# JeffWang987/MVSTER

Measured on AMD Instinct MI355X. Metric: depth-maps/sec (DTU 512×640, 5-view, 4-stage) at 1/2/4/8 MI355X, higher is better.
Workload: dtype f32; 1 GPU; DTU mid 512x640, 5 views, 4-stage cascade 8/8/4/4 hyp, B=1 eval, 1 depth map(s) per step per GPU; launch=hipGraph replay, parallelism=replicas x1, depth_maps_in_flight_per_gpu=2

## Files before the change

### include/mvster_hip.h

```cpp
#ifndef MVSTER_HIP_H
#define MVSTER_HIP_H

#ifdef __cplusplus
extern "C" {
#endif

#define MVSTER_OK 0
#define MVSTER_ERR_NULL (-1)
#define MVSTER_ERR_SHAPE (-2)
#define MVSTER_ERR_UNSUPPORTED (-3)
#define MVSTER_ERR_LAUNCH (-4)

int mvster_relative_projection(const float* proj_matrices, float* rt, int B, int N, void* stream);

int mvster_relative_projection_multi(const float* const* proj_matrices, int nstage, float* rt, int B, int N,
                                     void* stream);

int mvster_pack_images(const float* const* imgs, int N, float* out, int B, int H, int W, void* stream);

int mvster_pack_images_u8(const unsigned char* imgs, float* out, int V, int H, int W, void* stream);

int mvster_load_pack_images_u8(const unsigned char* buf, long buf_bytes, const int* desc_host, const int* desc, const void* tables,
                               long table_words, float* out, unsigned char* out_u8, int V, int Hd, int Wd, void* stream);

int mvster_forward_prologue(const float* const* imgs, int N, float* packed, int B, int H, int W,
                            const float* const* proj_matrices, int nstage, float* rt, const float* depth_values, int ndv,
                            float* hypo, int D, int h, int w, int inverse, void* stream);

int mvster_warp_agg_fwd(const float* ref_feat, const float* src_feat, const float* rt, const float* hypo,
                        float* out, float* wsum_out, int B, int NV, int C, int G, int D, int h, int w, int Hs,
                        int Ws, long ref_batch_stride, long src_view_stride, long src_batch_stride, int group_cor,
                        int attn_fuse_d, float attn_temp, int variant, void* stream);

int mvster_warp_agg_fwd_indexed(const float* store, const int* views, const float* rt, const float* hypo, float* out,
                                float* wsum_out, int V, int B, int NV, int C, int G, int D, int h, int w, int group_cor,
                                int attn_fuse_d, float attn_temp, int variant, void* stream);

int mvster_warp_agg_fwd_counted(const float* ref_feat, const float* src_feat, const float* rt, const float* hypo,
                                float* out, float* wsum_out, int B, int NV, int C, int G, int D, int h, int w, int Hs,
                                int Ws, long ref_batch_stride, long src_view_stride, long src_batch_stride, int group_cor,
                                int attn_fuse_d, float attn_temp, int variant, const int* nsrc, void* stream);
int mvster_warp_agg_fwd_indexed_counted(const float* store, const int* views, const float* rt, const float* hypo, float* out,
                                        float* wsum_out, int V, int B, int NV, int C, int G, int D, int h, int w,
                                        int group_cor, int attn_fuse_d, float attn_temp, int variant, const int* nsrc,
                                        void* stream);

int mvster_gather_views(const float* store, const int* views, float* out, int V, int B, int N, long map_floats, void* stream);

int mvster_warp_agg_fwd_sched(const float* ref_feat, const float* src_feat, const float* rt, const float* inv_min,
                              const float* inv_max, const float* depth_values, int ndv, float* hypo_out, float* out,
                              float* wsum_out, int B, int NV, int C, int G, int D, int h, int w, int Hs, int Ws,
                              long ref_batch_stride, long src_view_stride, long src_batch_stride, int attn_fuse_d,
                              float attn_temp, int mode, void* stream);

int mvster_warp_agg_bwd(const float* ref_feat, const float* src_feat, const float* rt, const float* hypo,
                        const float* out, const float* wsum, const float* grad_out, float* grad_ref,
                        float* grad_src, float* windows, int* win_org, int B, int NV, int C, int G, int D, int h, int w,
                        int Hs, int Ws, long ref_batch_stride, long src_view_stride, long src_batch_stride, int group_cor,
                        int attn_fuse_d, float attn_temp, void* stream);
int mvster_warp_agg_bwd_scratch(int B, int NV, int C, int G, int D, int h, int w, int attn_fuse_d, long* window_floats,
                                long* origin_ints);

int mvster_warp_agg_bwd_sorted_scratch(int B, int NV, int C, int D, int h, int w, int Hs, int Ws, long* rec_floats, long* ints);
int mvster_warp_agg_bwd_sorted(const float* ref_feat, const float* src_feat, const float* rt, const float* hypo,
                               const float* out, const float* wsum, const float* grad_out, float* grad_ref, float* grad_src,
                               float* rec, int* ints, int B, int NV, int C, int G, int D, int h, int w, int Hs, int Ws,
                               long ref_batch_stride, long src_view_stride, long src_batch_stride, int group_cor,
                               int attn_fuse_d, float attn_temp, void* stream);

int mvster_init_range(const float* depth_values, int ndv, float* out, int B, int D, int h, int w, int inverse,
                      void* stream);

int mvster_schedule_inverse_range(const float* inv_min, const float* inv_max, float* out, int B, int D, int h,
                                  int w, void* stream);

int mvster_schedule_range(const float* cur_depth, const float* interval, float* out, int B, int D, int h, int w,
                          void* stream);

int mvster_select_depth(const float* logits, const float* feat, const float* prob_w, const float* prob_b, int CF,
                        const float* hypo, float* attn, float* depth, float* conf, float* inv_min, float* inv_max,
                        float* logits_out, int B, int D, int h, int w, float split_itv, void* stream);

int mvster_select_depth_bwd(const float* attn, const float* gattn, const float* feat, const float* prob_w, float* dfeat,
                            float* partial, int B, int D, int h, int w, int CF, void* stream);

int mvster_upsample_bilinear(const float* in, float* out, int B, int hi, int wi, int ho, int wo, void* stream);

int mvster_upsample_bilinear_multi(const float* const* ins, float* const* outs, const int* his, const int* wis, int n, int B,
                                   int ho, int wo, void* stream);

int mvster_conv_mfma(const float* in, const float* wpk, const float* scale, const float* shift, const float* skip,
                     const float* zeros, const float* prob_w, const float* prob_b, float* out, const int* geom,
                     int ngeom, const long* woff, int cin, int mt, int nt, int variant, void* stream);

int mvster_conv_small(const float* in, const float* w, const float* scale, const float* shift, const float* skip,
                      float* out, int NB, int H, int W, int cin, int relu, void* stream);

int mvster_conv_narrow(const float* in, const float* w, const float* scale, const float* shift, const float* skip,
                       float* out, int NB, int H, int W, int cin, int relu, int mt, int wpc, void* stream);

int mvster_conv_narrow4(const float* in, const float* w, const float* scale, const float* shift, float* out, int NB, int H,
                        int W, int relu, int mt, int wpc, void* stream);

int mvster_conv_narrow_pair(const float* in, const float* w1, const float* scale1, const float* shift1, const float* w2,
                            const float* scale2, const float* shift2, float* out, int NB, int H, int W, int relu1, int relu2,
                            int wpc, void* stream);

int mvster_deconv_small(const float* in, const float* w, const float* scale, const float* shift, const float* skip,
                        const float* prob_w, const float* prob_b, float* out, int NB, int Hi, int Wi, int cin,
                        int cout, int relu, void* stream);

int mvster_deconv_select(const float* in, const float* w, const float* scale, const float* shift, const float* skip,
                         const float* prob_w, const float* prob_b, const float* hypo, float* attn, float* depth, float* conf,
                         float* inv_min, float* inv_max, float* logits_out, int B, int D, int Hi, int Wi, int cin, int relu,
                         float split_itv, void* stream);

int mvster_fpn_tail_gather(const float* G, const float* vb, float* P, float* workspace, int NB, int H, int W,
                           int CO, void* stream);

int mvster_fpn_tail_gather_bwd(const float* gP, float* gG, int NB, int H, int W, int CO, int pitch, void* stream);

int mvster_fpn_lateral_up(const float* x, const float* A, const float* bias, const float* q, float* out, int NB,
                          int H, int W, int CI, int CO, void* stream);

int mvster_fpn_tail_fused(const float* x, const float* A, const float* bias, const float* q, const float* vb, float* P,
                          int NB, int H, int W, int CI, void* stream);

int mvster_pack_conv_weights(const float* w, float* wpk, int cout, int cin, int cin_pad, int kd, int kh, int kw, long s_n,
                             long s_c, long s_z, long s_y, long s_x, int flip, void* stream);

int mvster_pack_wino_weights(const float* w, float* wpk, int cout, int cin, int cin_pad, int kd, long s_n, long s_c, long s_z,
                             long s_y, long s_x, int flip, void* stream);

int mvster_pack_wino_batch(const void* descs, int ndesc, int total_blocks, void* stream);

int mvster_pack_conv_weights_classes(const float* w, float* wpk, int cout, int cin, int cin_pad, int ktot, int nclass,
                                     const int* ntaps, const long* woff, const int* taps, void* stream);

int mvster_conv_wgrad(const float* x, const float* gy, float* partial, int nblk, int B, int Di, int Hi, int Wi, int CI,
                      int Do, int Ho, int Wo, int CO, int kd, int kh, int kw, int sd, int sh, int sw, int pd, int ph,
                      int pw, int packed, void* stream);

int mvster_conv_wgrad_slots(int CI, int CO, int kd, int kh, int kw, int sd, int sh, int sw, int pd, int ph, int pw, int packed);

int mvster_conv_wgrad_finish(const float* partial, float* dw, int nblk, int ngrp, int cop, int width, int ntaps, int cip,
                             int co_lim, int ci_lim, int swap, int flip, void* stream);

int mvster_conv_wgrad_finish_batch(const void* recs, int count, void* stream);

int mvster_bn_relu_fwd(const float* x, const float* scale, const float* shift, const float* skip, float* y, long rows,
                       int C, int relu, int groups, void* stream);
int mvster_bn_slots(long rows, int C, int groups);
int mvster_bn_relu_bwd_reduce(const float* x, const float* gy, const float* scale, const float* shift, const float* mean,
                              const float* rstd, float* partial, float* sums, float* dgamma, float* dbeta, int* ticket,
                              long rows, int C, int relu, int groups, void* stream);
int mvster_bn_relu_bwd_apply(const float* x, const float* gy, const float* scale, const float* shift, const float* mean,
                             const float* rstd, const float* sums, float* dx, long rows, int C, int relu, int groups,
                             int frozen, void* stream);

int mvster_col_sum(const float* x, float* partial, float* out, int* ticket, long rows, int C, void* stream);

int mvster_bn_train_slots(long rows, int C, int groups);
int mvster_bn_train_fwd(const float* x, const float* weight, const float* bias, float* running_mean, float* running_var,
                        long* num_batches_tracked, const float* skip, float* partial, float* y, float* out, long rows, int C,
                        int relu, int groups, float eps, float momentum, void* stream);
int mvster_bn_train_bwd(const float* x, const float* gy, const float* pack, float* partial, float* dgamma, float* dbeta, float* dx,
                        long rows, int C, int relu, int groups, void* stream);

int mvster_upsample2x_cl_fwd(const float* in, float* out, int B, int h, int w, int C, void* stream);
int mvster_upsample2x_cl_bwd(const float* gout, float* gin, int B, int h, int w, int C, void* stream);
int mvster_upsample2x_nearest_cl(const float* in, float* out, int B, int h, int w, int C, int backward, void* stream);

int mvster_sinkhorn(const float* attn, const float* hypo, const float* gt, float* loss_pix, float* jac, int B, int D,
                    long HW, int iters, float eps, void* stream);
int mvster_sinkhorn_continuous(const float* attn, const float* hypo, const float* gt, const float* mask, float* loss_pix,
                               float* jac, int B, int D, long HW, int iters, float eps, void* stream);

int mvster_stage_loss_terms(const float* hypo, const float* gt, const float* mask, const float* loss_pix,
                            const float* mono, float* terms, int B, int D, long HW, int inverse_depth, void* stream);

int mvster_geo_filter(const float* depth_ref, const float* depth_src, const double* ref_mats, const double* view_mats,
                      int* mask_sum, float* depth_sum, unsigned char* view_mask, float* view_depth, float* x_src,
                      float* y_src, int NS, int H, int W, float pix_thres, float rel_thres, void* stream);


int mvster_geo_scene_blocks(int R, int H, int W);

int mvster_geo_scene_filter(const float* depth, const float* confidence, const int* pairs, const int* ref_view,
                            const double* ref_mats, const double* view_mats, int* mask_sum, double* depth_avg,
// ... 78 lines not shown
```

### mvster_amd/_lib.py

```python
import ctypes
import os

_HERE = os.path.dirname(os.path.abspath(__file__))
LIB_PATH = os.environ.get("MVSTER_LIB") or os.path.join(_HERE, "csrc", "libmvster_hip.so")

ERR_NULL, ERR_SHAPE, ERR_UNSUPPORTED, ERR_LAUNCH = -1, -2, -3, -4
ERRORS = {-1: "NULL pointer", -2: "bad shape", -3: "unsupported channel/tile combination", -4: "kernel launch failed"}

_f = ctypes.c_void_p
_i = ctypes.c_int
_l = ctypes.c_long
_fl = ctypes.c_float

SIGNATURES = {
    "mvster_relative_projection": [_f, _f, _i, _i, _f],
    "mvster_relative_projection_multi": [_f, _i, _f, _i, _i, _f],
    "mvster_pack_images": [_f, _i, _f, _i, _i, _i, _f],
    "mvster_pack_images_u8": [_f, _f, _i, _i, _i, _f],
    "mvster_load_pack_images_u8": [_f, _l, _f, _f, _f, _l, _f, _f, _i, _i, _i, _f],
    "mvster_forward_prologue": [_f, _i, _f, _i, _i, _i, _f, _i, _f, _f, _i, _f, _i, _i, _i, _i, _f],
    "mvster_warp_agg_fwd": [_f, _f, _f, _f, _f, _f] + [_i] * 9 + [_l] * 3 + [_i, _i, _fl, _i, _f],
    "mvster_warp_agg_fwd_indexed": [_f, _f, _f, _f, _f, _f] + [_i] * 10 + [_fl, _i, _f],
    "mvster_warp_agg_fwd_counted": [_f, _f, _f, _f, _f, _f] + [_i] * 9 + [_l] * 3 + [_i, _i, _fl, _i, _f, _f],
    "mvster_warp_agg_fwd_indexed_counted": [_f, _f, _f, _f, _f, _f] + [_i] * 10 + [_fl, _i, _f, _f],
    "mvster_gather_views": [_f, _f, _f, _i, _i, _i, _l, _f],
    "mvster_warp_agg_fwd_sched": [_f] * 6 + [_i, _f, _f, _f] + [_i] * 9 + [_l] * 3 + [_i, _fl, _i, _f],
    "mvster_warp_agg_bwd": [_f] * 11 + [_i] * 9 + [_l] * 3 + [_i, _i, _fl, _f],
    "mvster_warp_agg_bwd_scratch": [_i] * 8 + [_f, _f],
    "mvster_warp_agg_bwd_sorted_scratch": [_i] * 8 + [_f, _f],
    "mvster_warp_agg_bwd_sorted": [_f] * 11 + [_i] * 9 + [_l] * 3 + [_i, _i, _fl, _f],
    "mvster_init_range": [_f, _i, _f, _i, _i, _i, _i, _i, _f],
    "mvster_schedule_inverse_range": [_f, _f, _f, _i, _i, _i, _i, _f],
    "mvster_schedule_range": [_f, _f, _f, _i, _i, _i, _i, _f],
    "mvster_select_depth": [_f, _f, _f, _f, _i, _f, _f, _f, _f, _f, _f, _f, _i, _i, _i, _i, _fl, _f],
    "mvster_select_depth_bwd": [_f, _f, _f, _f, _f, _f, _i, _i, _i, _i, _i, _f],
    "mvster_upsample_bilinear": [_f, _f, _i, _i, _i, _i, _i, _f],
    "mvster_upsample_bilinear_multi": [_f, _f, _f, _f, _i, _i, _i, _i, _f],
    "mvster_conv_mfma": [_f, _f, _f, _f, _f, _f, _f, _f, _f, _f, _i, _f, _i, _i, _i, _i, _f],
    "mvster_conv_small": [_f, _f, _f, _f, _f, _f, _i, _i, _i, _i, _i, _f],
    "mvster_conv_narrow": [_f, _f, _f, _f, _f, _f, _i, _i, _i, _i, _i, _i, _i, _f],
    "mvster_conv_narrow4": [_f, _f, _f, _f, _f, _i, _i, _i, _i, _i, _i, _f],
    "mvster_conv_narrow_pair": [_f, _f, _f, _f, _f, _f, _f, _f, _i, _i, _i, _i, _i, _i, _f],
    "mvster_deconv_select": [_f] * 14 + [_i] * 6 + [_fl, _f],
    "mvster_deconv_small": [_f, _f, _f, _f, _f, _f, _f, _f, _i, _i, _i, _i, _i, _i, _f],
    "mvster_fpn_tail_gather": [_f, _f, _f, _f, _i, _i, _i, _i, _f],
    "mvster_fpn_lateral_up": [_f, _f, _f, _f, _f, _i, _i, _i, _i, _i, _f],
    "mvster_fpn_tail_fused": [_f, _f, _f, _f, _f, _f, _i, _i, _i, _i, _f],
    "mvster_fpn_tail_gather_bwd": [_f, _f, _i, _i, _i, _i, _i, _f],
    "mvster_pack_conv_weights": [_f, _f] + [_i] * 6 + [_l] * 5 + [_i, _f],
    "mvster_pack_wino_weights": [_f, _f, _i, _i, _i, _i, _l, _l, _l, _l, _l, _i, _f],
    "mvster_pack_wino_batch": [_f, _i, _i, _f],
    "mvster_pack_conv_weights_classes": [_f, _f, _i, _i, _i, _i, _i, _f, _f, _f, _f],
    "mvster_conv_wgrad": [_f, _f, _f] + [_i] * 20 + [_f],
    "mvster_conv_wgrad_slots": [_i] * 12,
    "mvster_bn_relu_fwd": [_f, _f, _f, _f, _f, _l, _i, _i, _i, _f],
    "mvster_conv_wgrad_finish": [_f, _f] + [_i] * 10 + [_f],
    "mvster_bn_slots": [_l, _i, _i],
    "mvster_col_sum": [_f, _f, _f, _f, _l, _i, _f],
    "mvster_bn_train_slots": [_l, _i, _i],
    "mvster_bn_train_fwd": [_f] * 10 + [_l, _i, _i, _i, _fl, _fl, _f],
    "mvster_bn_train_bwd": [_f] * 7 + [_l, _i, _i, _i, _f],
    "mvster_conv_wgrad_finish_batch": [_f, _i, _f],
    "mvster_bn_relu_bwd_reduce": [_f] * 11 + [_l, _i, _i, _i, _f],
    "mvster_bn_relu_bwd_apply": [_f] * 8 + [_l, _i, _i, _i, _i, _f],
    "mvster_upsample2x_cl_fwd": [_f, _f, _i, _i, _i, _i, _f],
    "mvster_upsample2x_cl_bwd": [_f, _f, _i, _i, _i, _i, _f],
    "mvster_upsample2x_nearest_cl": [_f, _f, _i, _i, _i, _i, _i, _f],
    "mvster_sinkhorn": [_f, _f, _f, _f, _f, _i, _i, _l, _i, _fl, _f],
    "mvster_sinkhorn_continuous": [_f, _f, _f, _f, _f, _f, _i, _i, _l, _i, _fl, _f],
    "mvster_stage_loss_terms": [_f, _f, _f, _f, _f, _f, _i, _i, _l, _i, _f],
    "mvster_stage_loss_slots": [_l],
    "mvster_stage_loss_fwd": [_f] * 9 + [_i, _i, _l, _i, _fl, _fl, _fl, _f],
    "mvster_stage_loss_bwd": [_f] * 6 + [_fl, _fl, _f, _f, _i, _i, _l, _f],
    "mvster_mono_depth_fwd": [_f] * 5 + [_i, _l, _f],
    "mvster_mono_depth_bwd": [_f] * 6 + [_i, _l, _f],
    "mvster_upcat_fwd": [_f, _f, _f, _i, _i, _i, _i, _i, _f],
    "mvster_upcat_bwd": [_f, _f, _f, _i, _i, _i, _i, _i, _f],
    "mvster_fine_weights_fwd": [_f] * 6 + [_i, _i, _i, _f],
    "mvster_fine_weights_bwd": [_f] * 9 + [_i, _i, _i, _f],
    "mvster_fused_adam": [_f, _f, _f, _f, _i, _f, _f, _f, _f] + [ctypes.c_double] * 4 + [_f],
    "mvster_geo_filter": [_f] * 10 + [_i, _i, _i, _fl, _fl, _f],
    "mvster_geo_scene_blocks": [_i, _i, _i],
    "mvster_geo_scene_filter": [_f] * 13 + [_i] * 5 + [_fl, _i, _fl, _fl, _f],
    "mvster_geo_scene_filter_dynamic": [_f] * 14 + [_i] * 5 + [_fl, _i, _fl, _fl, _f],
    "mvster_geo_scene_emit": [_f] * 5 + [_i, _f, _f, _f, _l, _i, _i, _i, _i, _f],
    "mvster_voxel_thin_blocks": [_l],
    "mvster_voxel_thin_insert": [_f, _l, _fl, _f, _f, _l, _f, _f, _f, _f],
    "mvster_voxel_thin_emit": [_f, _f, _l, _fl, _i] + [_f] * 8 + [_l, _f],
    "mvster_depth_metrics_slots": [_l],
    "mvster_depth_metrics": [_f] * 5 + [_i, _i, _l, _f, _f, _f, _f],
    "mvster_pooled_metrics": [_f] * 5 + [_i, _i, _l, _f, _f, _f, _f],
    "mvster_scalar_accumulate": [_f, _i, _f, _f, _f],
    "mvster_scalar_gather_accumulate": [_f, _i, _f, _f, _f, _f],
    "mvster_scalar_reset": [_f, _i, _f, _f],
    "mvster_mfma_probe": [_f, _f, _f, _f],
    "mvster_gather_batch": [_f, _i, _i, _f],
    "mvster_last_kernel": [],
    "mvster_build_flags": [],
}
RESTYPES = {"mvster_last_kernel": ctypes.c_char_p}

_lib = None


def load():
    global _lib
    if _lib is None:
        if not os.path.exists(LIB_PATH):
            raise RuntimeError(
                "mvster_amd: %s not found. Build it with `python -c 'import __graft_entry__ as g; g.build()'` "
                "(hipcc --offload-arch=gfx950). There is no PyTorch fallback for the HIP path." % LIB_PATH)
        lib = ctypes.CDLL(LIB_PATH)
        lax = bool(os.environ.get("MVSTER_LIB")) and bool(os.environ.get("MVSTER_LIB_LAX"))
        for name, argtypes in SIGNATURES.items():
            if lax and not hasattr(lib, name):
                continue
            fn = getattr(lib, name)
            fn.argtypes = argtypes
            fn.restype = RESTYPES.get(name, ctypes.c_int)
        _lib = lib
    return _lib


def check(rc, what):
    if rc != 0:
# ... 11 lines not shown
```

### mvster_amd/conv_plan.py

```python
import ctypes

import numpy as np
import torch

from . import _lib, ops

GEOM = ("B", "Di", "Hi", "Wi", "Do", "Ho", "Wo", "DoF", "HoF", "WoF", "sd", "sh", "sw", "cout", "ntile_total", "relu",
        "skip_mode", "osd", "osh", "osw", "nclass")
GEOM_CLASS = ("kd", "kh", "kw", "pd", "ph", "pw", "od", "oh", "ow", "nsteps")

SKIP_NONE, SKIP_ADD, SKIP_UPSAMPLE_ADD = 0, 1, 2


def _pack_gemm(wk):
    K, N = wk.shape
    Kp, Np = (K + 15) // 16 * 16, (N + 15) // 16 * 16
    full = wk.new_zeros(Kp, Np)
    full[:K, :N] = wk
    return full.view(Kp // 16, 4, 4, Np // 16, 16).permute(0, 3, 1, 4, 2).contiguous().view(-1), Kp // 16


def fold_bn(bn, cout, device):
    if bn is None:
        return torch.ones(cout, device=device), torch.zeros(cout, device=device)
    scale = bn.weight.detach() / torch.sqrt(bn.running_var.detach() + bn.eps)
    shift = bn.bias.detach() - bn.running_mean.detach() * scale
    return scale.float(), shift.float()


_TUNING = None


def _tuning():
    global _TUNING
    if _TUNING is None:
        import json
        import os
        path = os.environ.get("MVSTER_TUNING") or os.path.join(os.path.dirname(os.path.abspath(__file__)), "tuning_gfx950.json")
        try:
            with open(path) as f:
                _TUNING = json.load(f)
        except (OSError, ValueError):
            _TUNING = {}
    return _TUNING


def layer_signature(layer, B, Di, Hi, Wi, skip_mode):
    return "%s%d-%d_k%dx%dx%d_s%dx%dx%d_%dx%dx%dx%d_sk%d" % (
        "T" if layer.transposed else "C", layer.cin, layer.cout, *layer.kernel, *layer.stride, B, Di, Hi, Wi, skip_mode)


FAMILY_REACH = 2.0
_FAMILIES = None
_SIG = None


def _families():
    global _FAMILIES, _SIG
    if _FAMILIES is None:
        import math
        import re
        _SIG = re.compile(r"^([CT]\d+-\d+_k\dx\dx\d_s\dx\dx\d)_(\d+)x(\d+)x(\d+)x(\d+)_sk([012])$")
        fam = {}
        for sig, val in _tuning().items():
            m = _SIG.match(sig)
            if not m:
                continue
            B, D, H, W = (int(m.group(i)) for i in (2, 3, 4, 5))
            fam.setdefault((m.group(1), int(m.group(6))), []).append((math.log2(B * D * H * W), math.log2(D), math.log2(B), list(val)))
        for lst in fam.values():
            lst.sort(key=lambda e: e[:3])
        _FAMILIES = fam
    return _FAMILIES


def tuned_choice(layer, B, Di, Hi, Wi, skip_mode):
    import math
    sig = layer_signature(layer, B, Di, Hi, Wi, skip_mode)
    hit = _tuning().get(sig)
    if hit:
        return hit, "exact"
    if skip_mode == SKIP_ADD:
        hit = _tuning().get(sig[:-1] + "0")
        if hit:
            return hit, "exact (without skip)"
    lst = _families().get((sig[:sig.index("_", sig.index("_s") + 1)], skip_mode))
    if lst:
        lv, ld, lb = math.log2(max(1, B * Di * Hi * Wi)), math.log2(max(1, Di)), math.log2(max(1, B))
        d, val = min(((abs(e[0] - lv) + abs(e[1] - ld) + 0.25 * abs(e[2] - lb), e[3]) for e in lst), key=lambda t: t[0])
        if d <= FAMILY_REACH:
            return list(val), "family"
    return None, None


FUSE_TAIL = True
FUSE_SELECT = True
LDS_BUDGET = 12 * 256 * 16
FORCE_VARIANT = None
TPERS16_MIN_VOXELS = 40960
FUSE_CONV0 = True
NARROW_PAIR_WPC = 1
NARROW_PAIR_MIN_PIXELS = 512 * 14 * 64
NARROW_MIN_VOXELS = 64 * 256


def _lds_plan(B, Do, Ho, Wo, kernel, stride, ntile_total):
    kd, kh, kw = kernel
    if kw not in (3, 5) or Wo < 24:
        return None
    for mt in (4, 2):
        ty = 2 * mt
        patch = kd * ((ty - 1) * stride[1] + kh) * (31 * stride[2] + kw) * 64
        if patch > LDS_BUDGET or (mt == 4 and Ho < 6):
            continue
        blocks = -(-Wo // 32) * -(-Ho // ty) * Do * B
        nt = max(n for n in (4, 2, 1) if n <= ntile_total and ntile_total % n == 0)
        while nt > 1 and blocks * (ntile_total // nt) < 512:
            nt //= 2
        return mt, nt
    return None


WINO_RING_INSTANCES = {(0, 1, 3), (0, 2, 3), (1, 2, 3), (2, 2, 3), (0, 4, 3), (1, 4, 3), (2, 4, 3),
                       (0, 4, 1), (1, 4, 1), (2, 4, 1), (0, 2, 1), (1, 2, 1), (2, 2, 1), (0, 1, 1), (2, 1, 1)}
WINO_INSTANCES = {(1, 1), (2, 1), (2, 2), (1, 2)}


def _wino_plan(layer, B, Do, Ho, Wo):
    tiles = B * Do * -(-Ho // 8) * -(-Wo // 32)
    kd = layer.kernel[0]
    if kd == 1 and layer.cin in (16, 32):
        nt = 2 if layer.ntile_total % 2 == 0 else 1
        if tiles * (layer.ntile_total // nt) >= 192:
            return 8 | (1 << 8), 2, nt
        return None
    nt = 2 if (layer.ntile_total % 2 == 0 and tiles * (layer.ntile_total // 2) >= 224) else 1
    if (1, layer.cin // 16, kd) not in WINO_RING_INSTANCES:
        nt = 1
    if tiles * (layer.ntile_total // nt) >= 160 and (0 if nt == 1 else 1, layer.cin // 16, kd) in WINO_RING_INSTANCES:
        return 9, 2, nt
    return None


def _tiles(M, ntile_total, nclass):
    best = None
    for nt in (5, 4, 3, 2, 1):
        if nt > ntile_total or ntile_total % nt:
            continue
        for mt in (4, 2, 1):
            waves = -(-M // (16 * mt)) * (ntile_total // nt) * nclass
            if waves >= 2048:
                return mt, nt
            if best is None or waves > best[0]:
                best = (waves, mt, nt)
    return best[1], best[2]


class ConvLayer:

    def __init__(self, weight, transposed, stride, padding, bn=None, bias=None, relu=False, cin_pad=None, prob=None):
        w = weight.detach().float()
        dev = w.device
        if w.dim() == 4:
            w = w.unsqueeze(2)
            stride = (1,) + tuple(stride)
            padding = (0,) + tuple(padding)
        self.transposed = transposed
        self.stride = tuple(stride)
        self.padding = tuple(padding)
        if transposed:
            cin, cout = w.shape[0], w.shape[1]
        else:
            cout, cin = w.shape[0], w.shape[1]
        self.cin = cin_pad or cin
        if self.cin not in (4, 8, 16, 32, 64, 80):
            raise RuntimeError("conv_mfma: unsupported input channel count %d" % self.cin)
        self.cout = cout
        self.relu = relu
        kd, kh, kw = w.shape[2:]
        self.kernel = (kd, kh, kw)
        self._cin_raw = cin
        self.classes, self.woff = self._class_table()
        self.wpk = None
        self.w_small = self.w_small4 = self.w_deconv = self.wpk_wino = self.wpk_b3 = self._b3_src = None
        self._pack(w)
# ... 322 lines not shown
            wpk = self.wpk_wino
        if (variant & 0xff) == 11:
            if self._b3_src is None or skip_mode == SKIP_UPSAMPLE_ADD or self.prob is not None:
                raise RuntimeError("conv_b3: layer not eligible")
            stamp = (self._b3_src._version, self._b3_src.data_ptr())
            if self.wpk_b3 is None or getattr(self, "_b3_stamp", None) != stamp:
                self.wpk_b3 = pack_b3(self._b3_src, self.cin, self.cout, self.kernel[0])
                self._b3_stamp = stamp
            wpk, nt = self.wpk_b3, 1
        rc = _lib.load().mvster_conv_mfma(
            x.data_ptr(), wpk.data_ptr(), self.scale.data_ptr(), self.shift.data_ptr(),
            None if skip is None else skip.data_ptr(), self.zeros.data_ptr(),
            None if self.prob is None else self.prob[0].data_ptr(), None if self.prob is None else self.prob[1].data_ptr(),
            out.data_ptr(), geom.ctypes.data_as(ctypes.c_void_p), int(geom.size), self.woff.ctypes.data_as(ctypes.c_void_p), self.cin,
            mt, nt, variant, ops._stream())
        if rc == _lib.ERR_UNSUPPORTED and tiles is None and variant != 0:
            mt, nt = _tiles(B * geom[4] * geom[5] * geom[6], self.ntile_total, len(self.classes))
            rc = _lib.load().mvster_conv_mfma(
                x.data_ptr(), self.wpk.data_ptr(), self.scale.data_ptr(), self.shift.data_ptr(),
                None if skip is None else skip.data_ptr(), self.zeros.data_ptr(),
                None if self.prob is None else self.prob[0].data_ptr(), None if self.prob is None else self.prob[1].data_ptr(),
                out.data_ptr(), geom.ctypes.data_as(ctypes.c_void_p), int(geom.size), self.woff.ctypes.data_as(ctypes.c_void_p),
                self.cin, mt, nt, 0, ops._stream())
        _lib.check(rc, "conv_mfma")
        return out

    def flops(self, B, Di, Hi, Wi):
        _, Do, Ho, Wo = self.out_shape(B, Di, Hi, Wi)
        kd, kh, kw = self.kernel
        if self.transposed:
            return 2 * B * Di * Hi * Wi * kd * kh * kw * self.cin * self.cout
        return 2 * B * Do * Ho * Wo * kd * kh * kw * self.cin * self.cout


def pack_b3(w, cin, cout, kd):
    if w.shape[1] != cin:
        w = torch.nn.functional.pad(w, (0, 0, 0, 0, 0, 0, 0, cin - w.shape[1]))
    w = w.reshape(cout, cin, kd, 9).float()
    w1 = w.to(torch.bfloat16)
    r = w - w1.float()
    w2 = r.to(torch.bfloat16)
    w3 = (r - w2.float()).to(torch.bfloat16)
    planes = torch.nn.functional.pad(torch.stack([w1, w2, w3]), (0, 1))
    ntw = 1 if cout == 16 else 2
    nsplit = cout // (16 * ntw)
    t = planes.reshape(3, nsplit, ntw, 16, cin // 16, 2, 8, kd, 5, 2).permute(7, 4, 1, 8, 2, 0, 9, 5, 3, 6)
    t = t.reshape(kd, cin // 16, nsplit, 5 * ntw * 3 * 64 * 8)
    return torch.nn.functional.pad(t, (0, 1024 * ntw * 8 - t.shape[-1])).contiguous()


def _cbr3d(m, **kw):
    return ConvLayer(m.conv.weight, False, m.conv.stride, m.conv.padding, bn=m.bn, relu=True, **kw)


def _up3d(seq, prob=None):
    ct, bn = seq[0], seq[1]
    return ConvLayer(ct.weight, True, ct.stride, ct.padding, bn=bn, relu=True, prob=prob)


def fused_conv11_select(L, t, c0, hypo, split_itv, inverse_depth, want_logits=False):
    B, D, hi, wi, _ = t.shape
    dev = t.device
    hypo = hypo.contiguous()
    attn = torch.empty(B, D, 2 * hi, 2 * wi, device=dev, dtype=torch.float32)
    depth = torch.empty(B, 2 * hi, 2 * wi, device=dev, dtype=torch.float32)
    conf = torch.empty_like(depth)
    imin = torch.empty_like(depth) if inverse_depth else None
    imax = torch.empty_like(depth) if inverse_depth else None
    lo = torch.empty_like(attn) if want_logits else None
    rc = _lib.load().mvster_deconv_select(
        t.data_ptr(), L.w_deconv.data_ptr(), L.scale.data_ptr(), L.shift.data_ptr(), c0.data_ptr(),
        L.prob[0].data_ptr(), L.prob[1].data_ptr(), hypo.data_ptr(), attn.data_ptr(), depth.data_ptr(), conf.data_ptr(),
        None if imin is None else imin.data_ptr(), None if imax is None else imax.data_ptr(),
        None if lo is None else lo.data_ptr(), B, D, hi, wi, L.cin, int(L.relu), float(split_itv), ops._stream())
    _lib.check(rc, "deconv_select")
    out = {"attn_weight": attn, "depth": depth, "conf": conf}
    if inverse_depth:
        out["inverse_min_depth"], out["inverse_max_depth"] = imin, imax
    if want_logits:
        out["logits"] = lo
    return out


class Reg2dPlan:

    def __init__(self, m, fuse_prob_into_conv11=True):
        self.conv0, self.conv1, self.conv2 = _cbr3d(m.conv0), _cbr3d(m.conv1), _cbr3d(m.conv2)
        self.conv3, self.conv4 = _cbr3d(m.conv3), _cbr3d(m.conv4)
        self.conv5, self.conv6 = _cbr3d(m.conv5), _cbr3d(m.conv6)
        self.conv7, self.conv9 = _up3d(m.conv7), _up3d(m.conv9)
        self.prob_w = m.prob.weight.detach().float().reshape(-1).contiguous()
        self.prob_b = m.prob.bias.detach().float().reshape(-1).contiguous()
        self.conv11 = _up3d(m.conv11, prob=(self.prob_w, self.prob_b) if fuse_prob_into_conv11 else None)
        self.fused_prob = not fuse_prob_into_conv11

    def layers(self):
        return [self.conv0, self.conv1, self.conv2, self.conv3, self.conv4, self.conv5, self.conv6, self.conv7,
                self.conv9, self.conv11]

    def __call__(self, x):
        c0 = self.conv0(x)
        c2 = self.conv2(self.conv1(c0))
        c4 = self.conv4(self.conv3(c2))
        t = self.conv6(self.conv5(c4))
        t = self.conv7(t, skip=c4, skip_mode=SKIP_ADD)
        t = self.conv9(t, skip=c2, skip_mode=SKIP_ADD)
        return self.conv11(t, skip=c0, skip_mode=SKIP_ADD)

    def select(self, x, hypo, split_itv, inverse_depth, want_logits=False):
        c0 = self.conv0(x)
        c2 = self.conv2(self.conv1(c0))
        c4 = self.conv4(self.conv3(c2))
        t = self.conv6(self.conv5(c4))
        t = self.conv7(t, skip=c4, skip_mode=SKIP_ADD)
        t = self.conv9(t, skip=c2, skip_mode=SKIP_ADD)
        L = self.conv11
        B, D, hi, wi, _ = t.shape
        if (FUSE_SELECT and L.w_deconv is not None and L.prob is not None and L.cin == 16 and FORCE_VARIANT in (None, 4)
                and 2 <= D <= 16 and t.is_contiguous() and c0.is_contiguous()):
            return fused_conv11_select(L, t, c0, hypo, split_itv, inverse_depth, want_logits)
        res = self.conv11(t, skip=c0, skip_mode=SKIP_ADD)
        if self.fused_prob:
            return ops.select_depth(hypo, split_itv, inverse_depth, feat_cl=res, prob_w=self.prob_w, prob_b=self.prob_b,
                                    want_logits=want_logits)
        return ops.select_depth(hypo, split_itv, inverse_depth, logits=res, want_logits=want_logits)

    def flops(self, B, D, h, w):
        tot, shp = 0, None
        dims = {"conv0": (D, h, w), "conv1": (D, h, w), "conv2": (D, h // 2, w // 2), "conv3": (D, h // 2, w // 2),
                "conv4": (D, h // 4, w // 4), "conv5": (D, h // 4, w // 4), "conv6": (D, h // 8, w // 8),
                "conv7": (D, h // 8, w // 8), "conv9": (D, h // 4, w // 4), "conv11": (D, h // 2, w // 2)}
        for k, (d_, h_, w_) in dims.items():
            tot += getattr(self, k).flops(B, d_, h_, w_)
        return tot + 2 * B * D * h * w * 8


class Reg3dPlan:

    def __init__(self, m):
        self.down_size = m.down_size
        self.conv0, self.conv1, self.conv2 = _cbr3d(m.conv0), _cbr3d(m.conv1), _cbr3d(m.conv2)
        if m.down_size >= 2:
            self.conv3, self.conv4 = _cbr3d(m.conv3), _cbr3d(m.conv4)
            self.conv9 = _up3d(m.conv9)
        if m.down_size >= 3:
            self.conv5, self.conv6 = _cbr3d(m.conv5), _cbr3d(m.conv6)
            self.conv7 = _up3d(m.conv7)
        self.conv11 = _up3d(m.conv11)
        self.prob = ConvLayer(m.prob.weight, False, m.prob.stride, m.prob.padding)
        self.fused_prob = False

    def __call__(self, x):
        c0 = self.conv0(x)
        c2 = self.conv2(self.conv1(c0))
        if self.down_size == 3:
            c4 = self.conv4(self.conv3(c2))
            t = self.conv6(self.conv5(c4))
            t = self.conv7(t, skip=c4, skip_mode=SKIP_ADD)
            t = self.conv9(t, skip=c2, skip_mode=SKIP_ADD)
        elif self.down_size == 2:
            t = self.conv4(self.conv3(c2))
            t = self.conv9(t, skip=c2, skip_mode=SKIP_ADD)
        else:
            t = c2
        t = self.conv11(t, skip=c0, skip_mode=SKIP_ADD)
        return self.prob(t).squeeze(-1)


def _cbr2d(m, **kw):
    c = m.conv
    return ConvLayer(c.weight, False, c.stride, c.padding, bn=m.bn, relu=m.relu, **kw)


def _plain2d(c):
    return ConvLayer(c.weight, False, c.stride, c.padding, bias=c.bias)


class FpnPlan:

    def __init__(self, m):
        self.conv0 = [_cbr2d(m.conv0[0], cin_pad=4), _cbr2d(m.conv0[1])]
        self.conv1 = [_cbr2d(l) for l in m.conv1]
        self.conv2 = [_cbr2d(l) for l in m.conv2]
        self.conv3 = [_cbr2d(l) for l in m.conv3]
        self.inner1 = _plain2d(m.inner1)
        self.out1, self.out2 = _plain2d(m.out1), _plain2d(m.out2)
        w2 = m.inner2.weight.detach().double()[:, :, 0, 0]
        b2 = m.inner2.bias.detach().double()
        self.mid_g, self.mid_c, self.mid_vb, _ = self._reassociate(m.out3, w2, b2)
        w3 = m.inner3.weight.detach().double()[:, :, 0, 0]
        b3 = m.inner3.bias.detach().double()
        self.tail_g, self.tail_c, self.tail_vb, wg4 = self._reassociate(m.out4, w3, b3)
        self.tail_a = (wg4 @ w2).float().contiguous()
        self.tail_ab = (wg4 @ b2).float().contiguous()

    @staticmethod
    def _reassociate(out, wi, bi):
        wo = out.weight.detach().double()
# ... 65 lines not shown
```

Before: 1161 depth-maps/s.

## Fuse conv7 and conv9 transposed-conv pair into one persistent MFMA kernel

Adds a persistent kernel that runs the two stride-2 transposed 3D convs (64->32 and 32->16) of the regularizer back to back per spatial tile. The intermediate 32-channel tensor stays in LDS instead of round-tripping through global memory, and one launch replaces two. Dedicated loader waves double-buffer input tiles via buffer-load-to-LDS, while compute waves run class-specialized MFMA loops. The cost is larger LDS use, halo recomputation at tile overlaps, and a fixed-shape path that only handles 64/32/16 channels.

```diff
diff --git a/include/mvster_hip.h b/include/mvster_hip.h
--- a/include/mvster_hip.h
+++ b/include/mvster_hip.h
@@ -105,6 +105,11 @@
 int mvster_conv_narrow_pair(const float* in, const float* w1, const float* scale1, const float* shift1, const float* w2,
                             const float* scale2, const float* shift2, float* out, int NB, int H, int W, int relu1, int relu2,
                             int wpc, void* stream);
+
+int mvster_conv_tpair(const float* in, const float* w7, const long* woff7, const int* nsteps7, const float* scale7,
+                      const float* shift7, const float* c4, const float* w9, const long* woff9, const int* nsteps9,
+                      const float* scale9, const float* shift9, const float* c2, float* out, int S, int Hi, int Wi, int cin,
+                      int cmid, int cout, int relu7, int relu9, int rows, void* stream);
 
 int mvster_deconv_small(const float* in, const float* w, const float* scale, const float* shift, const float* skip,
                         const float* prob_w, const float* prob_b, float* out, int NB, int Hi, int Wi, int cin,
diff --git a/mvster_amd/_lib.py b/mvster_amd/_lib.py
--- a/mvster_amd/_lib.py
+++ b/mvster_amd/_lib.py
@@ -41,6 +41,7 @@
     "mvster_conv_narrow": [_f, _f, _f, _f, _f, _f, _i, _i, _i, _i, _i, _i, _i, _f],
     "mvster_conv_narrow4": [_f, _f, _f, _f, _f, _i, _i, _i, _i, _i, _i, _f],
     "mvster_conv_narrow_pair": [_f, _f, _f, _f, _f, _f, _f, _f, _i, _i, _i, _i, _i, _i, _f],
+    "mvster_conv_tpair": [_f] * 14 + [_i] * 9 + [_f],
     "mvster_deconv_select": [_f] * 14 + [_i] * 6 + [_fl, _f],
     "mvster_deconv_small": [_f, _f, _f, _f, _f, _f, _f, _f, _i, _i, _i, _i, _i, _i, _f],
     "mvster_fpn_tail_gather": [_f, _f, _f, _f, _i, _i, _i, _i, _f],
diff --git a/mvster_amd/conv_plan.py b/mvster_amd/conv_plan.py
--- a/mvster_amd/conv_plan.py
+++ b/mvster_amd/conv_plan.py
@@ -101,6 +101,8 @@
 FUSE_CONV0 = True
 NARROW_PAIR_WPC = 1
 NARROW_PAIR_MIN_PIXELS = 512 * 14 * 64
+FUSE_UP_PAIR = True
+UP_PAIR_MIN_VOXELS = 0
 NARROW_MIN_VOXELS = 64 * 256
 
 
@@ -589,6 +591,41 @@
     return out
 
 
+def _is_up3(L, cin, cout):
+    return (L.transposed and L.kernel == (1, 3, 3) and L.stride == (1, 2, 2) and L.padding == (0, 1, 1) and L.cin == cin
+            and L.cout == cout and L.prob is None and len(L.classes) == 4 and L.wpk is not None)
+
+
+def fused_up_pair(L7, L9, t, c4, c2, rows=0, force=False):
+    if not force and (not FUSE_UP_PAIR or FORCE_VARIANT is not None):
+        return None
+    if t.dim() != 5 or not (_is_up3(L7, 64, 32) and _is_up3(L9, 32, 16)):
+        return None
+    B, D, hi, wi, C = t.shape
+    if (C != 64 or tuple(c4.shape) != (B, D, 2 * hi, 2 * wi, 32) or tuple(c2.shape) != (B, D, 4 * hi, 4 * wi, 16)
+            or not (t.is_cuda and t.is_contiguous() and c4.is_contiguous() and c2.is_contiguous())
+            or not (t.dtype == c4.dtype == c2.dtype == torch.float32) or L7.wpk.device != t.device):
+        return None
+    if not force and B * D * hi * wi < UP_PAIR_MIN_VOXELS:
+        return None
+    lib = _lib.load()
+    if not hasattr(lib, "mvster_conv_tpair"):
+        return None
+    for L in (L7, L9):
+        if getattr(L, "_nsteps_arr", None) is None:
+            L._nsteps_arr = np.asarray([c["nsteps"] for c in L.classes], dtype=np.int32)
+            L._woff_arr = np.ascontiguousarray(L.woff, dtype=np.int64)
+    out = torch.empty((B, D, 4 * hi, 4 * wi, 16), device=t.device, dtype=torch.float32)
+    vp = ctypes.c_void_p
+    rc = lib.mvster_conv_tpair(
+        t.data_ptr(), L7.wpk.data_ptr(), L7._woff_arr.ctypes.data_as(vp), L7._nsteps_arr.ctypes.data_as(vp), L7.scale.data_ptr(),
+        L7.shift.data_ptr(), c4.data_ptr(), L9.wpk.data_ptr(), L9._woff_arr.ctypes.data_as(vp), L9._nsteps_arr.ctypes.data_as(vp),
+        L9.scale.data_ptr(), L9.shift.data_ptr(), c2.data_ptr(), out.data_ptr(), B * D, hi, wi, L7.cin, L7.cout, L9.cout,
+        int(L7.relu), int(L9.relu), rows, ops._stream())
+    _lib.check(rc, "conv_tpair")
+    return out
+
+
 class Reg2dPlan:
 
     def __init__(self, m, fuse_prob_into_conv11=True):
@@ -610,17 +647,21 @@
         c2 = self.conv2(self.conv1(c0))
         c4 = self.conv4(self.conv3(c2))
         t = self.conv6(self.conv5(c4))
-        t = self.conv7(t, skip=c4, skip_mode=SKIP_ADD)
-        t = self.conv9(t, skip=c2, skip_mode=SKIP_ADD)
+        t = self._up_pair(t, c4, c2)
         return self.conv11(t, skip=c0, skip_mode=SKIP_ADD)
+
+    def _up_pair(self, t, c4, c2):
+        out = fused_up_pair(self.conv7, self.conv9, t, c4, c2)
+        if out is None:
+            out = self.conv9(self.conv7(t, skip=c4, skip_mode=SKIP_ADD), skip=c2, skip_mode=SKIP_ADD)
+        return out
 
     def select(self, x, hypo, split_itv, inverse_depth, want_logits=False):
         c0 = self.conv0(x)
         c2 = self.conv2(self.conv1(c0))
         c4 = self.conv4(self.conv3(c2))
         t = self.conv6(self.conv5(c4))
-        t = self.conv7(t, skip=c4, skip_mode=SKIP_ADD)
-        t = self.conv9(t, skip=c2, skip_mode=SKIP_ADD)
+        t = self._up_pair(t, c4, c2)
         L = self.conv11
         B, D, hi, wi, _ = t.shape
         if (FUSE_SELECT and L.w_deconv is not None and L.prob is not None and L.cin == 16 and FORCE_VARIANT in (None, 4)
diff --git a/mvster_amd/csrc/conv_tpair.hip b/mvster_amd/csrc/conv_tpair.hip
--- /dev/null
+++ b/mvster_amd/csrc/conv_tpair.hip
@@ -0,0 +1,354 @@
+#include "conv_args.hpp"
+#include "conv_tpair_geom.h"
+
+namespace mvconv {
+namespace {
+
+struct TpairArgs {
+    const float *in, *w7, *scale7, *shift7, *c4, *w9, *scale9, *shift9, *c2;
+    float* out;
+    int Hi, Wi;
+    int relu7, relu9;
+    unsigned tiles_x, tiles_y, ntiles;
+    unsigned in_bytes, mid_bytes, out_bytes;
+    unsigned mul[2], shr[2], one[2];
+};
+
+struct TpairPos { int s, vy0, vx0; };
+
+template <int CLS, int PLANE, int RS>
+__device__ __forceinline__ void tpair_mma7(f32x4v (&acc)[2], const f32x4v* patch, int abase, const f32x4v* wl7, int lane) {
+    constexpr int kw = (CLS & 1) + 1, nsteps = ((CLS >> 1) + 1) * kw * 4;
+    constexpr int wbase = CLS == 0 ? 0 : CLS == 1 ? 4 : CLS == 2 ? 12 : 20;
+    f32x4v w[2][2], av[2];
+    auto load = [&](int s, int b) {
+        const int tap = s >> 2, c = s & 3, dy = tap / kw, dx = tap - dy * kw;
+        w[b][0] = wl7[((wbase + s) * 2) * 64 + lane];
+        w[b][1] = wl7[((wbase + s) * 2 + 1) * 64 + lane];
+        av[b] = patch[abase + c * 2 * PLANE + dy * RS + dx * 2];
+    };
+    load(0, 0);
+#pragma unroll
+    for (int s = 0; s < nsteps; ++s) {
+        if (s + 1 < nsteps) load(s + 1, (s + 1) & 1);
+        __builtin_amdgcn_sched_barrier(0);
+#pragma unroll
+        for (int j = 0; j < 4; ++j) {
+            acc[0] = __builtin_amdgcn_mfma_f32_16x16x4f32(w[s & 1][0][j], av[s & 1][j], acc[0], 0, 0, 0);
+            acc[1] = __builtin_amdgcn_mfma_f32_16x16x4f32(w[s & 1][1][j], av[s & 1][j], acc[1], 0, 0, 0);
+        }
+    }
+}
+
+template <int CLS, int MPLANE, int MRS>
+__device__ __forceinline__ void tpair_mma9(f32x4v (&acc)[2], const f32x4v* midb, const int (&abase)[2], const f32x4v (&w9)[18]) {
+    constexpr int kw = (CLS & 1) + 1, nsteps = ((CLS >> 1) + 1) * kw * 2;
+    constexpr int wbase = CLS == 0 ? 0 : CLS == 1 ? 2 : CLS == 2 ? 6 : 10;
+    f32x4v av[2][2];
+    auto load = [&](int s, int b) {
+        const int tap = s >> 1, c = s & 1, dy = tap / kw, dx = tap - dy * kw;
+#pragma unroll
+        for (int m = 0; m < 2; ++m) av[b][m] = midb[abase[m] + c * 2 * MPLANE + dy * MRS + dx * 2];
+    };
+    load(0, 0);
+#pragma unroll
+    for (int s = 0; s < nsteps; ++s) {
+        if (s + 1 < nsteps) load(s + 1, (s + 1) & 1);
+        __builtin_amdgcn_sched_barrier(0);
+#pragma unroll
+        for (int j = 0; j < 4; ++j)
+#pragma unroll
+            for (int m = 0; m < 2; ++m) acc[m] = __builtin_amdgcn_mfma_f32_16x16x4f32(w9[wbase + s][j], av[s & 1][m][j], acc[m], 0, 0, 0);
+    }
+}
+
+template <int A>
+__global__ void __launch_bounds__(512) conv_tpair_kernel(TpairArgs a) {
+    using G = mvtpair::Geom<A>;
+    constexpr int PLANE = G::PLANE, RS = G::RS, NBLK = G::NBLK, MPLANE = G::MPLANE, MRS = G::MRS;
+    constexpr int BUF = 8 * PLANE;
+    constexpr int MBUF = 4 * MPLANE;
+    constexpr int NI = 8 * NBLK, NIW = (NI + 3) / 4;
+    constexpr int NS1 = mvtpair::slots1(A), NS2 = mvtpair::slots2(A);
+    extern __shared__ __attribute__((aligned(16))) float lds_raw[];
+    f32x4v* const lds = reinterpret_cast<f32x4v*>(lds_raw);
+    f32x4v* const scratch = lds + 2 * BUF;
+    f32x4v* const wl7 = scratch + 64;
+    f32x4v* const mid = wl7 + 72 * 64;
+
+    const int lane = threadIdx.x & 63;
+    const int wave8 = __builtin_amdgcn_readfirstlane(threadIdx.x >> 6);
+    const int wave = wave8 & 3;
+    const bool loader = wave8 >= 4;
+    const int lm = lane & 15, lq = lane >> 4;
+    auto decode_tile = [&](unsigned tile) -> TpairPos {
+        auto div = [&](unsigned n, int k) -> unsigned { return ((__umulhi(n, a.mul[k]) >> a.shr[k]) & ~a.one[k]) | (n & a.one[k]); };
+        const unsigned q = div(tile, 0), q2 = div(q, 1);
+        const mvtpair::Origin o = mvtpair::tile_origin((int)(q - q2 * a.tiles_y), (int)(tile - q * a.tiles_x), A);
+        return TpairPos{(int)q2, o.vy0, o.vx0};
+    };
+    const unsigned nwg = gridDim.x;
+    unsigned tile = xcd_remap(blockIdx.x, nwg);
+
+    if (loader) {
+        const __amdgpu_buffer_rsrc_t in_rsrc =
+            __builtin_amdgcn_make_buffer_rsrc(const_cast<float*>(a.in), (short)0, (int)a.in_bytes, 0x00020000);
+        unsigned dbase[NIW];
+        int dpos[NIW];
+#pragma unroll
+        for (int n = 0; n < NIW; ++n) {
+            const int i = wave + 4 * n;
+            const int c = i / (2 * NBLK), r = i - c * 2 * NBLK, pl = r / NBLK, blk = r - pl * NBLK;
+            const int s = blk * 64 + lane;
+            const int q1 = s & 1, pix = s >> 1;
+            const int prow = pix / mvtpair::kPatchW, px = pix - prow * mvtpair::kPatchW;
+            const bool valid = i < NI && prow < G::ROWS;
+            dpos[n] = px | (prow << 8);
+            dbase[n] = valid ? (unsigned)((prow * a.Wi + px) * 256 + (c * 16 + pl * 8 + q1 * 4) * 4) : 0x80000000u;
+        }
+        auto dma_tile = [&](const TpairPos& t, int buf, bool live) {
+            const unsigned origin = (unsigned)(((t.s * a.Hi + t.vy0) * a.Wi + t.vx0) * 256);
+            const mvtpair::Origin o{t.vy0, t.vx0};
+            f32x4v* const dst0 = lds + buf * BUF;
+#pragma unroll
+            for (int n = 0; n < NIW; ++n) {
+                const int i = wave + 4 * n;
+                const bool ok = live && mvtpair::in_inside(o, dpos[n] >> 8, dpos[n] & 255, a.Hi, a.Wi);
+                const unsigned off = ok ? dbase[n] + origin : 0x80000000u;
+                f32x4v* const dst = (NI % 4 == 0 || n + 1 < NIW || i < NI) ? dst0 + (i / NBLK) * PLANE + (i % NBLK) * 64 : scratch;
+                __builtin_amdgcn_raw_ptr_buffer_load_lds(in_rsrc, (lds_void*)dst, 16, off, 0, 0, 0);
+            }
+        };
+        if (tile < a.ntiles) dma_tile(decode_tile(tile), 0, true);
+        {
+            const __amdgpu_buffer_rsrc_t w7_rsrc =
+                __builtin_amdgcn_make_buffer_rsrc(const_cast<float*>(a.w7), (short)0, 72 * 1024, 0x00020000);
+            for (int i = wave; i < 72; i += 4) {
+                const unsigned off = (unsigned)(i * 1024 + lane * 16);
+                f32x4v* const dst = wl7 + i * 64;
+                __builtin_amdgcn_raw_ptr_buffer_load_lds(w7_rsrc, (lds_void*)dst, 16, off, 0, 0, 0);
+            }
+        }
+        asm volatile("s_waitcnt vmcnt(0)" ::: "memory");
+        __builtin_amdgcn_s_barrier();
+        for (int it = 0; tile < a.ntiles; tile += nwg, ++it) {
+            const bool has_next = tile + nwg < a.ntiles;
+            dma_tile(decode_tile(has_next ? tile + nwg : tile), (it & 1) ^ 1, has_next);
+            asm volatile("s_waitcnt vmcnt(0)" ::: "memory");
+            __builtin_amdgcn_s_barrier();
+        }
+        return;
+    }
+
+    f32x4v w9[18];
+#pragma unroll
+    for (int s = 0; s < 18; ++s) w9[s] = *reinterpret_cast<const f32x4v*>(a.w9 + (s * 64 + lane) * 4);
+    f32x4v sc7[2], sh7[2];
+#pragma unroll
+    for (int nt = 0; nt < 2; ++nt) {
+        sc7[nt] = *reinterpret_cast<const f32x4v*>(a.scale7 + nt * 16 + lq * 4);
+        sh7[nt] = *reinterpret_cast<const f32x4v*>(a.shift7 + nt * 16 + lq * 4);
+    }
+    const f32x4v sc9 = *reinterpret_cast<const f32x4v*>(a.scale9 + lq * 4), sh9 = *reinterpret_cast<const f32x4v*>(a.shift9 + lq * 4);
+    const mvtpair::Work wk1 = mvtpair::phase1_work(A, wave), wk2 = mvtpair::phase2_work(A, wave);
+    const __amdgpu_buffer_rsrc_t c4_rsrc =
+        __builtin_amdgcn_make_buffer_rsrc(const_cast<float*>(a.c4), (short)0, (int)a.mid_bytes, 0x00020000);
+    const __amdgpu_buffer_rsrc_t c2_rsrc =
+        __builtin_amdgcn_make_buffer_rsrc(const_cast<float*>(a.c2), (short)0, (int)a.out_bytes, 0x00020000);
+    const __amdgpu_buffer_rsrc_t out_rsrc = __builtin_amdgcn_make_buffer_rsrc(a.out, (short)0, (int)a.out_bytes, 0x00020000);
+    const int lsel = (lq >> 1), lpar = (lq & 1);
+    const int Hm = 2 * a.Hi, Wm = 2 * a.Wi, Wo = 4 * a.Wi;
+
+    f32x4v sk1[NS1][2];
+    auto fetch_c4 = [&](const TpairPos& t) {
+        const mvtpair::Origin org{t.vy0, t.vx0};
+#pragma unroll
+        for (int sl = 0; sl < NS1; ++sl) {
+            const int row = wk1.row[sl], cls = wk1.cls[sl];
+            if (cls < 0) continue;
+            const int py = cls >> 1, px = cls & 1;
+            const bool inside = mvtpair::voxel_inside(org, row, lm, a.Hi, a.Wi);
+            const unsigned cbase = (unsigned)((((t.s * Hm + 2 * (t.vy0 + row) + py) * Wm + 2 * (t.vx0 + lm) + px) * 32 + lq * 4)) * 4u;
+#pragma unroll
+            for (int nt = 0; nt < 2; ++nt) {
+                const unsigned off = inside ? cbase + (unsigned)(nt * 64) : 0x80000000u;
+                sk1[sl][nt] = __builtin_bit_cast(f32x4v, __builtin_amdgcn_raw_buffer_load_b128(c4_rsrc, off, 0, 0));
+            }
+        }
+    };
+    auto phase1 = [&](const TpairPos& t, const f32x4v* patch, f32x4v* midb) {
+        const mvtpair::Origin org{t.vy0, t.vx0};
+#pragma unroll
+        for (int sl = 0; sl < NS1; ++sl) {
+            const int row = wk1.row[sl], cls = wk1.cls[sl];
+            if (cls < 0) continue;
+            const int py = cls >> 1, px = cls & 1;
+            const bool inside = mvtpair::voxel_inside(org, row, lm, a.Hi, a.Wi);
+            const int abase = row * RS + lm * 2 + lsel * PLANE + lpar;
+            const int mbase = (2 * row + py) * MRS + (2 * lm + px) * 2 + lsel * MPLANE + lpar;
+            f32x4v acc[2];
+            acc[0] = acc[1] = (f32x4v){0.f, 0.f, 0.f, 0.f};
+            switch (cls) {
+                case 0: tpair_mma7<0, PLANE, RS>(acc, patch, abase, wl7, lane); break;
+                case 1: tpair_mma7<1, PLANE, RS>(acc, patch, abase, wl7, lane); break;
+                case 2: tpair_mma7<2, PLANE, RS>(acc, patch, abase, wl7, lane); break;
+                default: tpair_mma7<3, PLANE, RS>(acc, patch, abase, wl7, lane); break;
+            }
+#pragma unroll
+            for (int nt = 0; nt < 2; ++nt) {
+                f32x4v v = acc[nt];
+#pragma unroll
+                for (int j = 0; j < 4; ++j) {
+                    v[j] = fmaf(v[j], sc7[nt][j], sh7[nt][j]);
+                    if (a.relu7) v[j] = fmaxf(v[j], 0.0f);
+                    v[j] += sk1[sl][nt][j];
+                    v[j] = inside ? v[j] : 0.0f;
+                }
+                midb[nt * 2 * MPLANE + mbase] = v;
+            }
+        }
+    };
+    f32x4v sk2[NS2][2];
+    unsigned ooff[NS2][2];
+    auto fetch_c2 = [&](const TpairPos& t) {
+        const mvtpair::Origin org{t.vy0, t.vx0};
+#pragma unroll
+        for (int sl = 0; sl < NS2; ++sl) {
+            const int row = wk2.row[sl], cls = wk2.cls[sl];
+            if (cls < 0) continue;
+            const int py = cls >> 1, px = cls & 1;
+#pragma unroll
+            for (int m = 0; m < 2; ++m) {
+                const int mc = m * 16 + lm;
+                const unsigned off = (unsigned)((((t.s * 2 * Hm + 2 * (2 * t.vy0 + row) + py) * Wo + 2 * (2 * t.vx0 + mc) + px) * 16 + lq * 4)) * 4u;
+                ooff[sl][m] = mvtpair::out_owned(org, row, mc, a.Hi, a.Wi) ? off : 0x80000000u;
+                sk2[sl][m] = __builtin_bit_cast(f32x4v, __builtin_amdgcn_raw_buffer_load_b128(c2_rsrc, ooff[sl][m], 0, 0));
+            }
+        }
+    };
+    auto phase2 = [&](const f32x4v* midb) {
+#pragma unroll
+        for (int sl = 0; sl < NS2; ++sl) {
+            const int row = wk2.row[sl], cls = wk2.cls[sl];
+            if (cls < 0) continue;
+            int abase[2];
+#pragma unroll
+            for (int m = 0; m < 2; ++m) abase[m] = row * MRS + (m * 16 + lm) * 2 + lsel * MPLANE + lpar;
+            f32x4v acc[2];
+            acc[0] = acc[1] = (f32x4v){0.f, 0.f, 0.f, 0.f};
+            switch (cls) {
+                case 0: tpair_mma9<0, MPLANE, MRS>(acc, midb, abase, w9); break;
+                case 1: tpair_mma9<1, MPLANE, MRS>(acc, midb, abase, w9); break;
+                case 2: tpair_mma9<2, MPLANE, MRS>(acc, midb, abase, w9); break;
+                default: tpair_mma9<3, MPLANE, MRS>(acc, midb, abase, w9); break;
+            }
+#pragma unroll
+            for (int m = 0; m < 2; ++m) {
+                f32x4v v = acc[m];
+#pragma unroll
+                for (int j = 0; j < 4; ++j) {
+                    v[j] = fmaf(v[j], sc9[j], sh9[j]);
+                    if (a.relu9) v[j] = fmaxf(v[j], 0.0f);
+                    v[j] += sk2[sl][m][j];
+                }
+                __builtin_amdgcn_raw_buffer_store_b128(__builtin_bit_cast(u32x4v, v), out_rsrc, ooff[sl][m], 0, MV_STORE_AUX);
+            }
+        }
+    };
+
+    TpairPos pos = decode_tile(tile);
+    fetch_c4(pos);
+    asm volatile("s_waitcnt vmcnt(0)" ::: "memory");
+    __builtin_amdgcn_s_barrier();
+    phase1(pos, lds, mid);
+    fetch_c2(pos);
+    for (int it = 0; tile < a.ntiles; tile += nwg, ++it) {
+        __builtin_amdgcn_fence(__ATOMIC_RELEASE, "workgroup");
+        __builtin_amdgcn_s_waitcnt(0xc07f);
+        __builtin_amdgcn_s_barrier();
+        __builtin_amdgcn_fence(__ATOMIC_ACQUIRE, "workgroup");
+        const bool has_next = tile + nwg < a.ntiles;
+        const TpairPos next = decode_tile(has_next ? tile + nwg : tile);
+        if (has_next) fetch_c4(next);
+        phase2(mid + (it & 1) * MBUF);
+        if (has_next) {
+            phase1(next, lds + ((it & 1) ^ 1) * BUF, mid + ((it & 1) ^ 1) * MBUF);
+            fetch_c2(next);
+        }
+    }
+}
+
+template <int A>
+int launch_tpair(TpairArgs& a, int S, hipStream_t s) {
+    using G = mvtpair::Geom<A>;
+    const size_t lds = (size_t)G::LDS_F4 * 16;
+    static_assert((size_t)G::LDS_F4 * 16 <= 160 * 1024, "the pair's LDS budget");
+    auto kern = conv_tpair_kernel<A>;
+    static unsigned long attr_done = 0;
+    if (!allow_big_lds(reinterpret_cast<const void*>(kern), attr_done)) return MVSTER_ERR_LAUNCH;
+    const int ncu = num_cus();
+    if (ncu <= 0) return MVSTER_ERR_LAUNCH;
+    a.tiles_x = (unsigned)mvtpair::tiles_x(a.Wi);
+    a.tiles_y = (unsigned)mvtpair::tiles_y(a.Hi, A);
+    const long ntiles = (long)a.tiles_x * a.tiles_y * S;
+    if (ntiles >= (1L << 30)) return MVSTER_ERR_SHAPE;
+    a.ntiles = (unsigned)ntiles;
+    const unsigned divisors[2] = {a.tiles_x, a.tiles_y};
+    for (int i = 0; i < 2; ++i) {
+        find_divisor(divisors[i], a.mul[i], a.shr[i]);
+        a.one[i] = divisors[i] == 1 ? ~0u : 0u;
+    }
+    const long gmax = ncu;
+    const long rounds = (ntiles + gmax - 1) / gmax;
+    const long gx = (ntiles + rounds - 1) / rounds;
+    MV_NOTE_KERNEL("conv_tpair_kernel<%d>", A);
+    hipLaunchKernelGGL(kern, dim3((unsigned)gx, 1, 1), dim3(512), lds, s, a);
+    return mv_check_launch();
+}
+
+}
+}
+
+extern "C" int mvster_conv_tpair(const float* in, const float* w7, const long* woff7, const int* nsteps7, const float* scale7,
+                                 const float* shift7, const float* c4, const float* w9, const long* woff9, const int* nsteps9,
+                                 const float* scale9, const float* shift9, const float* c2, float* out, int S, int Hi, int Wi,
+                                 int cin, int cmid, int cout, int relu7, int relu9, int rows, void* stream) {
+    using namespace mvconv;
+    if (cin != 64 || cmid != 32 || cout != 16) return MVSTER_ERR_UNSUPPORTED;
+    if (!in || !w7 || !woff7 || !nsteps7 || !scale7 || !shift7 || !c4 || !w9 || !woff9 || !nsteps9 || !scale9 || !shift9 || !c2 || !out)
+        return MVSTER_ERR_NULL;
+    if (S <= 0 || Hi <= 0 || Wi <= 0) return MVSTER_ERR_SHAPE;
+    for (int c = 0; c < 4; ++c) {
+        const int taps = ((c >> 1) + 1) * ((c & 1) + 1);
+        if (nsteps7[c] != taps * 4 || nsteps9[c] != taps * 2) return MVSTER_ERR_UNSUPPORTED;
+        if (c > 0 && (woff7[c] != woff7[c - 1] + (long)nsteps7[c - 1] * 512 || woff9[c] != woff9[c - 1] + (long)nsteps9[c - 1] * 256))
+            return MVSTER_ERR_UNSUPPORTED;
+    }
+    if (rows < 0 || rows > 2) return MVSTER_ERR_UNSUPPORTED;
+    const long vox = (long)S * Hi * Wi;
+    if (vox >= (1L << 31) / 1024) return MVSTER_ERR_SHAPE;
+    TpairArgs a;
+    a.in = in;
+    a.w7 = w7 + woff7[0];
+    a.scale7 = scale7;
+    a.shift7 = shift7;
+    a.c4 = c4;
+    a.w9 = w9 + woff9[0];
+    a.scale9 = scale9;
+    a.shift9 = shift9;
+    a.c2 = c2;
+    a.out = out;
+    a.Hi = Hi;
+    a.Wi = Wi;
+    a.relu7 = relu7;
+    a.relu9 = relu9;
+    a.in_bytes = (unsigned)(vox * 256);
+    a.mid_bytes = (unsigned)(vox * 512);
+    a.out_bytes = (unsigned)(vox * 1024);
+    hipStream_t s = static_cast<hipStream_t>(stream);
+    if (rows == 0) {
+        const int ncu = num_cus();
+        rows = (long)mvtpair::tiles_x(Wi) * mvtpair::tiles_y(Hi, 1) * S <= ncu ? 1 : 2;
+    }
+    return rows == 1 ? launch_tpair<1>(a, S, s) : launch_tpair<2>(a, S, s);
+}
diff --git a/mvster_amd/csrc/conv_tpair_geom.h b/mvster_amd/csrc/conv_tpair_geom.h
--- /dev/null
+++ b/mvster_amd/csrc/conv_tpair_geom.h
@@ -0,0 +1,87 @@
+#pragma once
+
+#if defined(__HIPCC__)
+#define MVP_HD __host__ __device__ __forceinline__
+#else
+#define MVP_HD inline
+#endif
+
+namespace mvtpair {
+
+constexpr int kCols = 16;
+constexpr int kAdvX = 15;
+constexpr int kPatchW = kCols + 1;
+constexpr int kMidW = 2 * kCols;
+constexpr int kMidPitch = kMidW + 1;
+constexpr int kOwnW = 2 * kAdvX;
+
+template <int A>
+struct Geom {
+    static constexpr int ROWS = A + 1;
+    static constexpr int RS = kPatchW * 2;
+    static constexpr int USED = ROWS * RS;
+    static constexpr int NBLK = (USED + 63) / 64;
+    static constexpr int PLANE = ((NBLK * 64 + 7) & ~7) + 4;
+    static constexpr int MROWS = 2 * A + 1;
+    static constexpr int MRS = kMidPitch * 2;
+    static constexpr int MPLANE = ((MROWS * MRS + 7) & ~7) + 4;
+    static constexpr int LDS_F4 = 2 * 8 * PLANE + 64 + 72 * 64 + 2 * 4 * MPLANE;
+};
+
+MVP_HD int tiles_x(int Wi) { return (Wi + kAdvX - 1) / kAdvX; }
+MVP_HD int tiles_y(int Hi, int A) { return (Hi + A - 1) / A; }
+
+struct Origin {
+    int vy0, vx0;
+};
+
+MVP_HD Origin tile_origin(int ty, int tx, int A) { return Origin{ty * A, tx * kAdvX}; }
+
+MVP_HD bool in_inside(Origin o, int prow, int pcol, int Hi, int Wi) { return o.vy0 + prow < Hi && o.vx0 + pcol < Wi; }
+
+MVP_HD bool voxel_inside(Origin o, int r, int c, int Hi, int Wi) { return o.vy0 + r < Hi && o.vx0 + c < Wi; }
+
+MVP_HD bool mid_zero(Origin o, int mr, int mc, int Hi, int Wi) { return 2 * o.vy0 + mr >= 2 * Hi || 2 * o.vx0 + mc >= 2 * Wi; }
+
+MVP_HD bool out_owned(Origin o, int mr, int mc, int Hi, int Wi) {
+    return mc < kOwnW && 2 * o.vy0 + mr < 2 * Hi && 2 * o.vx0 + mc < 2 * Wi;
+}
+
+struct Work {
+    int row[4], cls[4];
+};
+
+constexpr int slots1(int A) { return A == 2 ? 3 : 2; }
+constexpr int slots2(int A) { return A == 2 ? 4 : 2; }
+
+MVP_HD Work phase1_work(int A, int wave) {
+    Work w;
+    for (int i = 0; i < 4; ++i) { w.row[i] = 0; w.cls[i] = -1; }
+    if (A == 2) {
+        w.row[0] = w.row[1] = wave >> 1;
+        w.cls[0] = (wave & 1) ? 1 : 0;
+        w.cls[1] = (wave & 1) ? 2 : 3;
+        w.row[2] = 2;
+        w.cls[2] = wave == 1 ? 0 : wave == 3 ? 1 : -1;
+    } else {
+        w.cls[0] = wave == 0 ? 3 : wave == 1 ? 1 : wave == 2 ? 0 : -1;
+        w.row[1] = wave == 2 ? 0 : 1;
+        w.cls[1] = wave == 1 ? 0 : wave == 2 ? 2 : wave == 3 ? 1 : -1;
+    }
+    return w;
+}
+
+MVP_HD Work phase2_work(int A, int wave) {
+    Work w;
+    for (int i = 0; i < 4; ++i) { w.row[i] = 0; w.cls[i] = -1; }
+    if (A == 2) {
+        for (int i = 0; i < 4; ++i) { w.row[i] = wave; w.cls[i] = i; }
+    } else {
+        w.row[0] = w.row[1] = wave >> 1;
+        w.cls[0] = (wave & 1) ? 1 : 0;
+        w.cls[1] = (wave & 1) ? 2 : 3;
+    }
+    return w;
+}
+
+}
```

Measured after the change: 1170 depth-maps/s, median of 6. Within noise of the previous version (+0.7%).
